# AugmentariumLab/VolumeRenderer

Hardware: AMD Instinct MI355X
Metric: Mvoxels/s kd-tree compress+decode (higher is better)
Workload: dtype u8; 1 GPU; 2048x2048x1920 uint8 volume per GPU as 960 bricks of 256x256x128, rm_volume, tolerance 1, maxEpochs 2, VolumeKdtree build + levelCut

## Files before the change

volumerenderer_amd/csrc/brickset.h:

```cpp
#pragma once
#include "kd_common.h"
#include "../../include/vrhip.h"
#include <algorithm>
#include <string>
#include <vector>

namespace vr {

struct Stream2 {
    uint8_t *temp = nullptr;
    uint8_t *codes = nullptr;
    uint8_t *recon[3] = {nullptr, nullptr, nullptr};
    Ctrl *ctrl = nullptr;
    uint8_t *tree = nullptr;
    uint8_t *treeCompact = nullptr;
};

#define EST_R0_BUDGET 8
struct Switches {
    bool decodeWalk = false;
    bool decodeFineV1 = false;
    bool decodeQuad = false;
    bool noSkipBlocks = false;
    bool noUniformBlocks = false;
    bool estExactBounds = false;
    int estBudget = EST_R0_BUDGET;
    bool pyramidBoxes = false;
    bool indexPerBlock = false;
    bool noUniformDecode = false;
};

#define VR_LOD_SLOTS 4
struct LodSlot {
    int32_t *dev = nullptr;
    int32_t *host = nullptr;
    uint8_t *idxValCut = nullptr;
    uint32_t *decTables = nullptr;
    uint8_t *rankVals = nullptr;
    int64_t *obDev = nullptr;
    int64_t *obHost = nullptr;
    vr_pool_entry *tabHost = nullptr;
    int64_t tabCap = 0;
    hipEvent_t done = nullptr;
    bool pending = false;
};

struct BrickSet {
    int32_t B = 0;
    Switches sw;
    Geom g{};
    TilePlan tile{};
    RegionPlan region{};
    Pyr12Plan pyr12{};
    int32_t D = 0, maxDepth = 0;
    int32_t tolerance = 6, maxEpochs = 5, variant = 0;
    int32_t K = 0;
    int32_t Ds = 0;
    int64_t heapStride = 0;
    int64_t leafStride = 0;
// ... 111 lines not shown
```

volumerenderer_amd/csrc/capi.hip:

```cpp
#include "../../include/vrhip.h"
#include "brickset.h"
#include "raymarch.h"
#include <math.h>
#include <stdio.h>
#include <stdlib.h>
#include <string.h>
#include <algorithm>
#include <array>
#include <atomic>
#include <map>
#include <mutex>
#include <new>

using namespace vr;

struct vr_brickset { BrickSet s; };

#define HIPCHK(x) do { hipError_t e_ = (x); if (e_ != hipSuccess) return e_ == hipErrorOutOfMemory ? VR_ERR_OOM : VR_ERR_NO_DEVICE; } while (0)

static bool device_ok()
{
    int n = 0;
    hipError_t e = hipGetDeviceCount(&n);
    if ((e != hipSuccess || n <= 0) && getenv("VRHIP_DEBUG"))
// ... 183 lines not shown
}

static bool pow2(int64_t v) { return v > 0 && (v & (v - 1)) == 0; }

static bool misaligned16(const void *p) { return ((uintptr_t)p & 15) != 0; }

vr_status vr_brickset_create(vr_brickset **out, int32_t num_bricks, const int64_t dims[3], int32_t tolerance,
                             int32_t max_epochs, int32_t variant)
{
    if (!out || !dims || num_bricks <= 0) return VR_ERR_INVALID;
    if (tolerance < 0 || max_epochs < 0 || variant < 0 || variant > 2) return VR_ERR_INVALID;
    for (int k = 0; k < 3; ++k) if (dims[k] <= 0) return VR_ERR_INVALID;
    if (max_epochs > VR_MAX_EPOCHS) return VR_ERR_UNSUPPORTED;
    bool general = !pow2(dims[0]) || !pow2(dims[1]) || !pow2(dims[2]) || dims[0] > 1024 || dims[1] > 1024 || dims[2] > 1024;
    if (dims[0] > (1ll << 20) || dims[1] > (1ll << 20) || dims[2] > (1ll << 20) || dims[0] * dims[1] * dims[2] >= (1ll << 32))
        return VR_ERR_UNSUPPORTED;
    if (num_bricks > VR_MAX_BRICKS) return VR_ERR_UNSUPPORTED;
    if (!device_ok()) return VR_ERR_NO_DEVICE;
    vr_brickset *h = new (std::nothrow) vr_brickset();
    if (!h) return VR_ERR_OOM;
    BrickSet &b = h->s;
    b.B = num_bricks;
    {
        Switches &w = b.sw;
        w.decodeWalk = getenv("VRHIP_DECODE_WALK") != nullptr;
        w.decodeFineV1 = getenv("VRHIP_DECODE_FINE_V1") != nullptr;
        w.decodeQuad = getenv("VRHIP_DECODE_QUAD") != nullptr;
        w.noSkipBlocks = getenv("VRHIP_NO_SKIP_BLOCKS") != nullptr;
        w.noUniformBlocks = getenv("VRHIP_NO_UNIFORM_BLOCKS") != nullptr;
        w.noUniformDecode = getenv("VRHIP_NO_UNIFORM_DECODE") != nullptr;
        w.pyramidBoxes = getenv("VRHIP_PYRAMID_BOXES") != nullptr;
        w.indexPerBlock = getenv("VRHIP_INDEX_PER_BLOCK") != nullptr;
        w.estExactBounds = getenv("VRHIP_EST_EXACT_BOUNDS") != nullptr;
        if (const char *eb = getenv("VRHIP_EST_BUDGET")) { const int v = atoi(eb); if (v >= 0) w.estBudget = v; }
    }
    make_geom(b.g, dims);
    b.D = b.g.D;
    if (b.D > 31) { delete h; return VR_ERR_UNSUPPORTED; }
    b.idx64 = b.D > 28 || (getenv("VRHIP_FORCE_IDX64") && b.D >= 12);
    if (b.idx64) general = true;
    if (b.idx64 && num_bricks != 1 && b.D > 28) { delete h; return VR_ERR_UNSUPPORTED; }
    b.generalGeom = general;
    b.maxDepth = b.D + VR_CHAIN_LEVELS;
    b.tolerance = tolerance; b.maxEpochs = max_epochs; b.variant = variant;
    b.K = b.D < 6 ? b.D : 6;
    b.Ds = b.D - b.K;
    b.heapStride = (int64_t)1 << (b.D + 1);
    b.leafStride = (int64_t)1 << b.D;
    b.codeStride = ((b.heapStride + 15) / 16) * 4;
    b.reconStride = b.leafStride;
    const int64_t numMax = b.heapStride - 1 + VR_CHAIN_LEVELS * b.leafStride;
    b.treeCap = ((numMax + 15) / 16 + 2) * 4 + 256;
    if (b.D >= 12) {
        const int64_t gappedBytes = ((int64_t)1 << (b.D - 12)) * 2320 * 4 + 256;
        if (gappedBytes > b.treeCap) b.treeCap = gappedBytes;
    }
    b.nIdx = (int64_t)1 << b.Ds;
    make_plans(b.g, b.K, b.generalGeom, b.idx64, b.treeCap, b.tile, b.region, b.pyr12);
    vr_status rc = alloc_stream2(b, b.mid);
    if (rc == VR_OK) {
        hipError_t e = hipMalloc(&b.idxOff, (size_t)b.B * b.nIdx * sizeof(uint32_t));
        if (e == hipSuccess) e = hipMalloc(&b.idxVal, (size_t)b.B * b.nIdx);
        if (e == hipSuccess) e = hipMalloc(&b.idxValCut, (size_t)b.B * b.nIdx);
        if (e == hipSuccess && general) {
            const int grc = build_general_geometry(&b);
            if (grc != 0) e = grc == -3 ? hipErrorOutOfMemory : hipErrorUnknown;
        }
        const auto upload = [](uint32_t *dst, const std::vector<uint32_t> &v) {
            return hipMemcpy(dst, v.data(), v.size() * sizeof(uint32_t), hipMemcpyHostToDevice);
        };
        if (e == hipSuccess) e = hipMalloc(&b.lut, ((size_t)1 << b.K) * sizeof(uint32_t));
        if (e == hipSuccess && !general) e = upload(b.lut, make_lut(b.g, b.K));
        if (e == hipSuccess && !general) e = hipMalloc(&b.spread, (size_t)(b.g.X + b.g.Y + b.g.Z) * sizeof(uint32_t));
        if (e == hipSuccess && !general) e = upload(b.spread, make_spread(b.g));
        for (int i = 0; i < 8 && e == hipSuccess; ++i) e = hipEventCreate(&b.ev[i]);
        if (e != hipSuccess) rc = e == hipErrorOutOfMemory ? VR_ERR_OOM : VR_ERR_NO_DEVICE;
    }
    if (rc != VR_OK) { vr_brickset_destroy(h); return rc; }
    b.hostCtrl.resize(b.B);
    b.openTreeBytes.assign(b.B, -1);
    *out = h;
    return VR_OK;
}

vr_status vr_brickset_set_switch(vr_brickset *h, const char *name, int32_t value)
{
    if (!h || !name) return VR_ERR_INVALID;
    Switches &w = h->s.sw;
    const bool on = value != 0;
    if (!strcmp(name, "decode_walk")) w.decodeWalk = on;
    else if (!strcmp(name, "decode_fine_v1")) w.decodeFineV1 = on;
    else if (!strcmp(name, "decode_quad")) w.decodeQuad = on;
    else if (!strcmp(name, "no_skip_blocks")) w.noSkipBlocks = on;
    else if (!strcmp(name, "no_uniform_blocks")) w.noUniformBlocks = on;
    else if (!strcmp(name, "no_uniform_decode")) w.noUniformDecode = on;
    else if (!strcmp(name, "pyramid_boxes")) w.pyramidBoxes = on;
    else if (!strcmp(name, "index_per_block")) w.indexPerBlock = on;
    else if (!strcmp(name, "est_exact_bounds")) w.estExactBounds = on;
    else return VR_ERR_INVALID;
    return VR_OK;
}

vr_status vr_brickset_set_compaction(vr_brickset *h, int32_t on_build)
{
    if (!h) return VR_ERR_INVALID;
    h->s.compactOnBuild = on_build != 0;
    return VR_OK;
}

vr_status vr_debug_set(const char *name, int32_t value)
{
    if (!name) return VR_ERR_INVALID;
    if (!strcmp(name, "skip_grid_v1")) { vr::g_skipGridV1.store(value ? 1 : 0); return VR_OK; }
    if (!strcmp(name, "reslice_tile_w")) {
        if (value != 8 && value != 16 && value != 64) return VR_ERR_INVALID;
        vr::g_resliceTileLog2.store(value == 8 ? 3 : (value == 16 ? 4 : 6));
        return VR_OK;
    }
    if (!strcmp(name, "hist_plain")) { vr::g_histPlain.store(value ? 1 : 0); return VR_OK; }
    return VR_ERR_INVALID;
}

vr_status vr_brickset_set_error_tolerance(vr_brickset *h, int32_t tol)
{
    if (!h || tol < 0) return VR_ERR_INVALID;
    h->s.tolerance = tol;
    return VR_OK;
}
vr_status vr_brickset_set_max_epochs(vr_brickset *h, int32_t e)
{
    if (!h || e < 0) return VR_ERR_INVALID;
// ... 1316 lines not shown
```

volumerenderer_amd/csrc/host_plan.cpp:

```cpp
#include "host_plan.h"
#include "../../include/vrhip.h"
#include <string.h>
#include <algorithm>
#include <atomic>
#include <thread>

namespace vr {

static int next_split(int64_t ext[3], int d)
{
    int sd = d % 3, i = 0;
    while (ext[0] * ext[1] * ext[2] > 1 && ext[sd] == 1) sd = (d + ++i) % 3;
    ext[sd] /= 2;
    return sd;
}

void make_geom(Geom &g, const int64_t dims[3])
{
    memset(&g, 0, sizeof(g));
    g.X = (int32_t)dims[0]; g.Y = (int32_t)dims[1]; g.Z = (int32_t)dims[2];
    g.voxels = dims[0] * dims[1] * dims[2];
    int64_t ext[3] = {dims[0], dims[1], dims[2]};
    for (int k = 0; k < 3; ++k) { int n = 0; while (((int64_t)1 << (n + 1)) <= dims[k]) ++n; g.nb[k] = n; }
    g.D = g.nb[0] + g.nb[1] + g.nb[2];
// ... 335 lines not shown
        if (k.numActive <= 0) return;
        const int64_t tb = (k.numActive + 3) / 4;
        std::vector<uint8_t> &r = recs[(size_t)b];
        r.assign((size_t)archive_record_bytes(g.D, g.maxDepth, tb), 0);
        uint8_t *p = r.data();
        memcpy(p, k.dmap, (size_t)g.maxDepth + 1); p += pad16(g.maxDepth + 1);
        memcpy(p, k.topVal.data(), (size_t)2 << Dc); p += pad16((int64_t)2 << Dc);
        memcpy(p, k.blockOff.data(), (size_t)4 << Dc); p += pad16((int64_t)4 << Dc);
        memcpy(p, k.tree, (size_t)tb);
        dir[(size_t)b] = ArchiveEntry{0, tb, k.numActive, fnv1a64(r.data(), (int64_t)r.size())};
    });
    int64_t at = dirEnd;
    for (int b = 0; b < g.numBricks; ++b)
        if (!recs[(size_t)b].empty()) { dir[(size_t)b].offset = at; at += (int64_t)recs[(size_t)b].size(); }
    ArchiveHeader h;
    memset(&h, 0, sizeof(h));
    memcpy(h.magic, ARCHIVE_MAGIC, 8);
    h.version = 1; h.variant = (uint32_t)g.variant; h.numBricks = g.numBricks; h.D = g.D; h.maxDepth = g.maxDepth; h.fileBytes = at;
    for (int k = 0; k < 3; ++k) h.dims[k] = g.dims[k];
    bool ok = fwrite(&h, sizeof(h), 1, f) == 1 && fwrite(dir.data(), VR_ARCHIVE_ENTRY_BYTES, dir.size(), f) == dir.size();
    for (int b = 0; ok && b < g.numBricks; ++b)
        if (!recs[(size_t)b].empty()) ok = fwrite(recs[(size_t)b].data(), 1, recs[(size_t)b].size(), f) == recs[(size_t)b].size();
    return ok;
}

bool read_header(FILE *f, Header &h)
{
    if (fread(&h, VR_HEADER_BYTES, 1, f) != 1) return false;
    return h.maxDepth >= VR_CHAIN_LEVELS && h.maxDepth < VR_MAX_DEPTH && h.numActive > 0;
}

bool write_header(FILE *f, const Header &h) { return fwrite(&h, VR_HEADER_BYTES, 1, f) == 1; }

}

extern "C" vr_status vr_lod_select_error(const vr_brick_error *table, int32_t num_bricks, int32_t cut_lo, int32_t cut_hi,
                                         int64_t voxels_per_brick, const int32_t *cuts_in, int32_t max_abs_bound,
                                         double mean_sq_bound, int32_t *cuts_out)
{
    if (!table || !cuts_out || num_bricks < 1 || cut_lo < 0 || cut_lo > cut_hi || voxels_per_brick < 1) return VR_ERR_INVALID;
    if (max_abs_bound < 0 || mean_sq_bound != mean_sq_bound) return VR_ERR_INVALID;
    for (int32_t b = 0; cuts_in && b < num_bricks; ++b) if (cuts_in[b] < -1) return VR_ERR_INVALID;
    for (int32_t b = 0; b < num_bricks; ++b) {
        const int32_t h = cuts_in ? cuts_in[b] : cut_hi;
        int32_t pick = h;
        for (int32_t c = cut_lo; h >= 0 && c <= std::min(h, cut_hi); ++c) {
            const vr_brick_error &e = table[(int64_t)(c - cut_lo) * num_bricks + b];
            if (e.max_abs > (uint32_t)max_abs_bound) continue;
            if (mean_sq_bound >= 0.0 && !((double)e.sum_sq <= mean_sq_bound * (double)voxels_per_brick)) continue;
            pick = c;
            break;
        }
        cuts_out[b] = pick;
    }
    return VR_OK;
}

extern "C" vr_status vr_stream_block_table(const int64_t dims[3], const uint8_t *tree_host, int64_t tree_bytes, int64_t num_active,
                                           const uint8_t *dmap, int32_t map_len, uint32_t *block_off_out, uint8_t *top_val_out)
{
    if (!dims || !tree_host || !dmap || !block_off_out || !top_val_out || num_active <= 0) return VR_ERR_INVALID;
    for (int k = 0; k < 3; ++k) if (dims[k] <= 0 || dims[k] > (1ll << 20)) return VR_ERR_INVALID;
    if (dims[0] * dims[1] * dims[2] >= (1ll << 32)) return VR_ERR_UNSUPPORTED;
    vr::Geom g;
    vr::make_geom(g, dims);
    if (g.D > 31 || num_active >= (1ll << 32)) return VR_ERR_UNSUPPORTED;
// ... 32 lines not shown
```

volumerenderer_amd/csrc/host_plan.h:

```cpp
#pragma once
#include <stdint.h>
#include <stdio.h>
#include <array>
#include <functional>
#include <vector>

#if defined(__HIP__) || defined(__HIPCC__)
#define VR_HD __host__ __device__
#else
#define VR_HD
#endif

#define VR_MAX_DEPTH 40
#define VR_CHAIN_LEVELS 7
#define VR_IDX_DEAD 0xFFFFFFFFu

namespace vr {

struct Geom {
    int32_t D;
    int32_t nb[3];
    int32_t X, Y, Z;
    uint8_t axis[32];
    uint8_t bit[32];
// ... 15 lines not shown
    if (code == 1) { v += dist; return v > 255 ? 255 : v; }
    if (code == 2) { v -= dist; return v < 0 ? 0 : v; }
    return v;
}

VR_HD inline int cget(const uint8_t *C, int64_t i) { return (C[i >> 2] >> ((int)(i & 3) * 2)) & 3; }

void make_geom(Geom &g, const int64_t dims[3]);
std::vector<std::array<int, 3>> split_counts(const int64_t dims[3], int depths);
std::vector<uint32_t> make_lut(const Geom &g, int K);
std::vector<uint32_t> make_spread(const Geom &g);

constexpr int VR_RG_REGX = 128;

struct TilePlan {
    bool ok;
    int jx, jy, jz, tilesX, tilesY, tilesZ, ltx, lty;
    uint8_t kqBit[8];
};
struct RegionPlan {
    bool ok;
    int X, Y, lrx, lry, jx, nreg;
    int64_t voxels;
    uint32_t lanePos, parkP[4], parkS, gAddr[4], gByte, gOut[8], xRead[2], blkX, blkY, blkZ;
};
struct Pyr12Plan {
    bool use12;
    int ax, ay, az, swz, nbx, nby, lnbx, lnby;
    uint16_t sx[16];
    bool lines;
};
void make_plans(const Geom &g, int K, bool generalGeom, bool idx64, int64_t treeCap, TilePlan &tile, RegionPlan &region,
                Pyr12Plan &pyr12);

template <class Node, class Pruned, class Chain>
int walk_stream(int D, const uint8_t *tree, int64_t numActive, const uint8_t *dmap, int cut, Node node, Pruned pruned,
                Chain chain)
{
    int v[VR_MAX_DEPTH];
    int64_t pos = 0;
    int j = 0;
    uint32_t path = 0;
    while (true) {
        if (pos >= numActive) return -1;
        const int tok = cget(tree, pos);
        const int val = j == 0 ? dmap[0] : (j <= cut ? apply_code(v[j - 1], tok, dmap[j]) : v[j - 1]);
        v[j] = val;
        node(j, path, pos++, tok, val);
        bool terminal = tok == 3;
        if (terminal) pruned(j, path, val);
        else if (j == D) {
            for (int c = 1; c <= VR_CHAIN_LEVELS; ++c) {
                if (pos >= numActive) return -2;
                chain(path);
                if (cget(tree, pos++) == 3) break;
            }
            terminal = true;
        }
        if (terminal) {
            while (j > 0 && (path & 1u)) { path >>= 1; --j; }
            if (j == 0) break;
            path |= 1u;
        } else { ++j; path <<= 1; }
    }
    return pos == numActive ? 0 : -3;
}
// ... 116 lines not shown
```

volumerenderer_amd/csrc/kd_common.h:

```cpp
#pragma once
#include <hip/hip_runtime.h>
#include "host_plan.h"

namespace vr {

struct Ctrl {
    double currentDistance, currentError, currentDF, currentStepSize;
    double previousDistance, previousError, previousDF, previousStepSize;
    unsigned long long errMinus, errPlus;
    unsigned long long statL1;
    unsigned long long numActive;
    int32_t epoch;
    int32_t active;
    int32_t fillThisEpoch;
    int32_t cur, prev, pendingEqual;
    int32_t par, ra, rb;
    int32_t numReverts;
    int32_t maxErrBefore, maxErrAfter;
    int32_t estTbase;
    unsigned long long estS;
    uint32_t estC;
    int32_t estFallbacks;
    int32_t estSeg;
    int32_t estDone;
    int32_t emitOverflow;
    int32_t constBrick;
    int32_t constVal;
    int32_t roleDist[2], codesDist, finalReconDist, finalCodesDist;
    int32_t altValid, altDist, altSel;
    int32_t zeroRun;
    uint8_t distanceMap[VR_MAX_DEPTH + 8];
};

struct Enc { int code, recon, err; };
__host__ __device__ inline Enc encode_node(int t, int p, int d)
{
    int none = p > t ? p - t : t - p;
    int add = p + d > 255 ? 255 : p + d;
    int ae = add > t ? add - t : t - add;
    int sub = p - d < 0 ? 0 : p - d;
    int se = sub > t ? sub - t : t - sub;
    int m = none < ae ? none : ae;
    m = se < m ? se : m;
    Enc e;
    e.err = m;
    if (m == none) { e.code = 0; e.recon = p; }
    else if (m == ae) { e.code = 1; e.recon = add; }
    else { e.code = 2; e.recon = sub; }
    return e;
}

#ifdef __HIPCC__
// ... 105 lines not shown
```

volumerenderer_amd/csrc/kd_encode.hip:

```cpp
#include "brickset.h"
#include <math.h>
#include <stdio.h>
#include <stdlib.h>
#include <string.h>

namespace vr {

#define FILL_NODES_PER_BLOCK 1024
#define EMIT_RANKS_PER_BLOCK 256

template <bool FROM_VOXELS>
__global__ void __launch_bounds__(256)
k_pyramid(Geom g, int dLeaf, int L, const uint8_t *__restrict__ vox, const uint8_t *__restrict__ inMin,
          const uint8_t *__restrict__ inMax, int64_t inStride, uint8_t *__restrict__ temp, int64_t heapStride,
          uint8_t *__restrict__ tempRange, uint8_t *__restrict__ outMin, uint8_t *__restrict__ outMax,
          int64_t outStride, const uint32_t *__restrict__ srcIdx)
{
    __shared__ uint8_t smn[2][1024], smx[2][1024];
    const int brick = blockIdx.y;
    const uint32_t n = 1u << L;
    const uint32_t base = blockIdx.x << L;
    uint8_t *T = temp + (int64_t)brick * heapStride;
    uint8_t *TR = tempRange ? tempRange + (int64_t)brick * heapStride : nullptr;
    for (uint32_t i = threadIdx.x; i < n; i += blockDim.x) {
// ... 357 lines not shown
    int Dm2;
};
__device__ __forceinline__ bool skip_block(const SkipBlocks &sk, int brick, int d, uint32_t node)
{
    return sk.flag && d > sk.Dm2 && (sk.flag[(int64_t)brick * sk.nBlk + (node >> (10 + d - sk.Dm2))] & 2u) != 0u;
}

#ifndef VR_FLAGS_BATCHED
#define VR_FLAGS_BATCHED 1
#endif

__device__ inline int phys_buf(const Ctrl &c, int role) { return role == 0 ? c.ra : c.rb; }

__global__ void k_ctrl_init(Ctrl *ctrls, const uint8_t *rootMin, const uint8_t *rootMax, int64_t mmStride)
{
    Ctrl &c = ctrls[blockIdx.x];
    if (threadIdx.x) return;
    c.constBrick = 0; c.constVal = 0; c.zeroRun = 0;
    if (rootMin) {
        const int mn = rootMin[(int64_t)blockIdx.x * mmStride], mx = rootMax[(int64_t)blockIdx.x * mmStride];
        c.constBrick = mn == mx ? 1 : 0;
        c.constVal = mn;
    }
    c.currentDistance = c.currentError = c.currentDF = c.currentStepSize = 0.0;
    c.previousDistance = c.previousError = c.previousDF = c.previousStepSize = 0.0;
    c.errMinus = c.errPlus = 0;
    c.statL1 = 0;
    c.numActive = 0;
    c.epoch = 0; c.active = 0; c.fillThisEpoch = 0;
    c.cur = 0; c.prev = 1; c.pendingEqual = 0;
    c.par = 0; c.ra = 1; c.rb = 2;
    c.altValid = 0; c.altSel = 0; c.altDist = 0;
    c.numReverts = 0; c.maxErrBefore = 0; c.maxErrAfter = 0;
    c.estS = 0; c.estC = 0; c.estTbase = 0; c.estFallbacks = 0; c.estSeg = 0; c.estDone = 0; c.emitOverflow = 0;
    for (int i = 0; i < VR_MAX_DEPTH + 8; ++i) c.distanceMap[i] = 0;
}

#define EST_SEG 1024
#define EST_CAND 8
#define EST_ROUNDS 5
#define EST_HEAD 4096

#define est_at(ci, seg) (((int64_t)(ci) * summStride + (int64_t)(seg)) * 4)

__device__ __forceinline__ uint32_t wave_incl_scan_u32(uint32_t v, int lane)
{
    (void)lane;
    return wave_incl_scan_add_dpp(v);
}

__device__ __forceinline__ uint32_t lane_u32(uint32_t v, int l) { return (uint32_t)__builtin_amdgcn_readlane((int)v, l); }
__device__ __forceinline__ unsigned long long lane_u64(unsigned long long v, int l)
{
    return (unsigned long long)lane_u32((uint32_t)v, l) | ((unsigned long long)lane_u32((uint32_t)(v >> 32), l) << 32);
}

#define EST_STAGE_NODES 4096
__device__ inline void est_exact_chain(const uint8_t *__restrict__ T, const uint8_t *__restrict__ P, int d, uint32_t lo,
                                       uint32_t hi, unsigned long long &S, uint32_t &C, int lane, const SkipBlocks &sk, int brick,
                                       uint8_t *stage = nullptr)
{
    const uint32_t len = hi - lo;
    const bool staged = stage && d > 0 && len >= 64u && len <= (uint32_t)EST_STAGE_NODES && (len & 63u) == 0u && (lo & 31u) == 0u;
    const uint8_t *sT = stage, *sP = stage + EST_STAGE_NODES;
    if (staged) {
        for (uint32_t i = (uint32_t)lane * 16u; i < len; i += 1024u) *(uint4 *)(stage + i) = *(const uint4 *)(T + lo + i);
        for (uint32_t i = (uint32_t)lane * 16u; i < len / 2u; i += 1024u) *(uint4 *)(stage + EST_STAGE_NODES + i) = *(const uint4 *)(P + (lo >> 1) + i);
    }
    const bool sk0 = skip_block(sk, brick, d, lo);
    int tn = 0, pn = 0;
    if (staged) { tn = sT[lane]; pn = sP[lane >> 1]; }
    else { tn = (!sk0 && lo + lane < hi) ? T[lo + lane] : 0; pn = (!sk0 && lo + lane < hi && d > 0) ? P[(lo + lane) >> 1] : 0; }
    bool skipThis = sk0;
    for (uint32_t base = lo; base < hi; base += 64) {
// ... 4 lines not shown
        {
            const uint32_t i2 = i + 64;
            skipThis = base + 64 < hi && skip_block(sk, brick, d, base + 64);
            if (staged) {
                const uint32_t j2 = i2 - lo;
                tn = j2 < len ? sT[j2] : 0;
                pn = j2 < len ? sP[j2 >> 1] : 0;
            } else {
                tn = (!skipThis && i2 < hi) ? T[i2] : 0;
                pn = (!skipThis && i2 < hi && d > 0) ? P[i2 >> 1] : 0;
            }
        }
        if (skipped) continue;
        int pd = p > t ? p - t : t - p;
        bool forced = (t > p && 2 * t - p > 255) || (t < p && 2 * t < p);
        bool cand = valid && pd > 0;
        bool dec = cand && (forced || S < (unsigned long long)pd * (2ull * C + 1ull));
        unsigned long long mask = __ballot(dec);
        for (int it = 0; it < 65; ++it) {
            uint32_t cpre = __popcll(mask & ((1ull << lane) - 1ull));
            uint32_t v = dec ? (uint32_t)pd : 0u;
            uint32_t spre = wave_incl_scan_u32(v, lane) - v;
            bool nd = cand && (forced || (S + spre) < (unsigned long long)pd * (2ull * (C + cpre) + 1ull));
            unsigned long long nmask = __ballot(nd);
            dec = nd;
            if (nmask == mask) break;
            mask = nmask;
        }
        S += (uint32_t)__builtin_amdgcn_readlane((int)wave_incl_scan_add_dpp(dec ? (uint32_t)pd : 0u), 63);
        C += __popcll(mask);
    }
}

__device__ inline int est_window_base(long long T, int nc)
{
    long long b = T - (nc <= 4 ? 1 : 2);
    if (b < 0) b = 0;
    if (b > 256 - nc) b = 256 - nc;
    return (int)b;
}

__device__ inline void est_finish(Ctrl &c, unsigned long long S, uint32_t C, int maxEpochs)
{
    c.currentDistance = C > 0 ? round((double)S / (double)C) : 0.0;
    c.previousDistance = 0.0;
    c.previousStepSize = 255.0;
    c.previousError = 65025.0;
    c.epoch = 0;
    c.active = maxEpochs > 0 ? 1 : 0;
    c.fillThisEpoch = c.active;
    c.errMinus = c.errPlus = 0;
    c.cur = 0; c.prev = 1; c.pendingEqual = 0;
}

__global__ void __launch_bounds__(64)
k_est_head(int d, int maxEpochs, Ctrl *ctrls, const uint8_t *__restrict__ temp, int64_t heapStride, ReconBufs rb,
           int64_t leafStride, SkipBlocks sk)
{
    const int brick = blockIdx.x, lane = threadIdx.x;
    Ctrl &c = ctrls[brick];
    if (c.constBrick) return;
    const uint8_t *T = temp + (int64_t)brick * heapStride + ((int64_t)1 << d);
    const uint8_t *P = rb.b[c.par] + (int64_t)brick * leafStride;
    const uint32_t n = 1u << d;
    unsigned long long S = 0;
    uint32_t C = 0;
    __shared__ __attribute__((aligned(16))) uint8_t stage[EST_STAGE_NODES + EST_STAGE_NODES / 2];
    est_exact_chain(T, P, d, 0, n < EST_HEAD ? n : EST_HEAD, S, C, lane, sk, brick, stage);
    if (lane == 0) {
        if (n <= EST_HEAD) est_finish(c, S, C, maxEpochs);
        else {
            c.estS = S; c.estC = C;
            c.estSeg = EST_HEAD / EST_SEG;
            c.estDone = 0;
            c.estTbase = est_window_base((long long)(S / (2ull * C + 1ull)), 4);
        }
    }
}

__device__ __forceinline__ uint32_t seg_incl_scan_add_dpp(uint32_t v)
{
    v = row_incl_scan_add_dpp(v);
    return v + dpp_u32<0x142, 0xa>(0, v);
}
__device__ __forceinline__ int seg_max_i32_dpp(int v)
{
    v = row_max_i32_dpp(v);
    return max(v, (int)dpp_u32<0x142, 0xa>(0x80000000u, (uint32_t)v));
}
__device__ __forceinline__ int seg_min_i32_dpp(int v)
{
    v = row_min_i32_dpp(v);
    return min(v, (int)dpp_u32<0x142, 0xa>(0x7FFFFFFFu, (uint32_t)v));
}

template <bool QUADS>
__global__ void __launch_bounds__(256)
k_est_summ(int d, int nc, Ctrl *ctrls, const uint8_t *__restrict__ temp, int64_t heapStride, ReconBufs rb,
           int64_t leafStride, uint32_t *__restrict__ summ, int64_t summStride, SkipBlocks sk)
{
    constexpr int L = 32, SPW = 64 / L, NP = EST_SEG / 2 / L, TW = NP / 2, PW = NP / 4;
    const int brick = blockIdx.y, lane = threadIdx.x & 63, row = lane / L, rl = lane % L;
    const Ctrl &c = ctrls[brick];
    const uint32_t n = 1u << d;
    const int cConst = c.constBrick, cDone = c.estDone, cSeg = c.estSeg, cPar = c.par, cTbase = c.estTbase;
    if (cConst || cDone) return;
    const uint8_t *Tl = temp + (int64_t)brick * heapStride + ((int64_t)1 << d) + rl * (4 * TW);
    const uint8_t *Pl = (cPar == 0 ? rb.b[0] : (cPar == 1 ? rb.b[1] : rb.b[2])) + (int64_t)brick * leafStride + rl * (4 * PW);
    const uint32_t nseg = n / EST_SEG, step = gridDim.x * (4u * SPW);
    const uint32_t g0 = (uint32_t)cSeg + (blockIdx.x * 4u + (threadIdx.x >> 6)) * SPW;
    uint4 tN[TW / 4], pN[PW / 4];
    auto fetch = [&](uint32_t g) {
        const uint32_t s = g + (uint32_t)row;
        const bool live = s < nseg && !skip_block(sk, brick, d, s * EST_SEG);
#pragma unroll
        for (int j = 0; j < TW / 4; ++j) tN[j] = make_uint4(0, 0, 0, 0);
#pragma unroll
        for (int j = 0; j < PW / 4; ++j) pN[j] = make_uint4(0, 0, 0, 0);
        if (live) {
#pragma unroll
            for (int j = 0; j < TW / 4; ++j) tN[j] = ld16(Tl + (size_t)s * EST_SEG + 16 * j);
#pragma unroll
            for (int j = 0; j < PW / 4; ++j) pN[j] = ld16(Pl + (size_t)s * (EST_SEG / 2) + 16 * j);
        }
    };
    fetch(g0);
    const int Tbase = cTbase;
    uint32_t *out = summ + (int64_t)brick * summStride * (4 * EST_CAND);
    for (uint32_t g = g0; g < nseg; g += step) {
    uint32_t tw[TW], pw[PW];
#pragma unroll
    for (int j = 0; j < TW / 4; ++j) { tw[4 * j] = tN[j].x; tw[4 * j + 1] = tN[j].y; tw[4 * j + 2] = tN[j].z; tw[4 * j + 3] = tN[j].w; }
#pragma unroll
    for (int j = 0; j < PW / 4; ++j) { pw[4 * j] = pN[j].x; pw[4 * j + 1] = pN[j].y; pw[4 * j + 2] = pN[j].z; pw[4 * j + 3] = pN[j].w; }
    const uint32_t seg = g + (uint32_t)row;
    const bool segLive = seg < nseg;
    uint32_t mixed = 0;
    {
        const uint32_t t0 = __builtin_amdgcn_perm(0, tw[0], 0u), p0 = __builtin_amdgcn_perm(0, pw[0], 0u);
#pragma unroll
        for (int j = 0; j < TW; ++j) mixed |= tw[j] ^ t0;
#pragma unroll
        for (int j = 0; j < PW; ++j) mixed |= pw[j] ^ p0;
    }
    const bool uniform = __ballot(mixed != 0u) == 0ull;
    constexpr int NU = QUADS ? 1 : NP, NQ = QUADS ? TW : 1;
    vr_s16x2 pd[NU], h[NU];
    uint32_t anyPd = 0;
    uint32_t pd4[NQ], hi[NQ], anyF = 0;
    vr_s16x2 pm = (vr_s16x2)(0);
    const auto unpack4 = [&](const int q) {
        const uint32_t psel = (uint32_t)((2 * q) & 3);
        const vr_s16x2 P2 = pk_s(__builtin_amdgcn_perm(0, pw[q >> 1], 0x0c000c00u | psel | ((psel + 1u) << 16)));
        const vr_s16x2 Te = pk_s(__builtin_amdgcn_perm(0, tw[q], 0x0c020c00u)), To = pk_s(__builtin_amdgcn_perm(0, tw[q], 0x0c030c01u));
        const vr_s16x2 de = Te - P2, dO = To - P2;
        const vr_s16x2 pe = __builtin_elementwise_max(de, (vr_s16x2)(0) - de), po = __builtin_elementwise_max(dO, (vr_s16x2)(0) - dO);
        const uint32_t fb = __builtin_amdgcn_perm(pk_u(To + dO), pk_u(Te + de), 0x07030501u);
        pd4[q] = __builtin_amdgcn_perm(pk_u(po), pk_u(pe), 0x06020400u);
        hi[q] = ((fb << 7) | pd4[q]) & 0x80808080u;
        anyF |= fb;
// ... 76 lines not shown
                bmin = __builtin_elementwise_min(bmin, pk_mad(cc, two2, low));
            }
        }
        } else
#pragma unroll
        for (int k = 0; k < NP; ++k) {
            const vr_s16x2 dm = (__builtin_elementwise_min(Th2, h[k]) - pd[k]) >> 15;
            low = dm * (pd[k] - w2) + low;
            cc -= dm;
            if (k < NP - 1) {
                amax = __builtin_elementwise_max(amax, low);
                bmin = __builtin_elementwise_min(bmin, pk_mad(cc, two2, low));
            }
        }
        const int low1 = low.x, low2 = low.y, cc1 = cc.x, cc2 = cc.y;
        lowT = low1 + low2; ccT = cc1 + cc2;
        a = max((int)amax.x, max((int)amax.y, 0) + low1);
        b = min((int)bmin.x, min((int)bmin.y, 0) + low1 + 2 * cc1);
        }
        const uint32_t sT = (uint32_t)(2 * Th * ccT - lowT);
        const uint32_t packed = sT | ((uint32_t)ccT << 20);
        const uint32_t incl = seg_incl_scan_add_dpp(packed), excl = incl - packed;
        const int s0 = (int)(excl & 0xFFFFFu), c0 = (int)(excl >> 20);
        a += 2 * Th * c0 - s0;
        b += 2 * (Th + 1) * c0 - s0;
        a = seg_max_i32_dpp(a);
        b = seg_min_i32_dpp(b);
        if (segLive && rl == L - 1)
            *(uint4 *)(out + est_at(ci, seg)) = make_uint4(incl & 0xFFFFFu, incl >> 20, (uint32_t)a, (uint32_t)b);
    }
    }
}

__global__ void __launch_bounds__(64)
k_est_walk(int d, int maxEpochs, int nc, int ncNext, int lastRound, int budget, Ctrl *ctrls, const uint8_t *__restrict__ temp, int64_t heapStride, ReconBufs rb,
           int64_t leafStride, const uint32_t *__restrict__ summ, int64_t summStride, SkipBlocks sk)
{
    const int brick = blockIdx.x, lane = threadIdx.x;
    Ctrl &c = ctrls[brick];
    const uint8_t *T = temp + (int64_t)brick * heapStride + ((int64_t)1 << d);
    const uint8_t *P = rb.b[c.par] + (int64_t)brick * leafStride;
    const uint32_t n = 1u << d, nseg = n / EST_SEG;
    const uint32_t *sm = summ + (int64_t)brick * summStride * (4 * EST_CAND);
    if (c.constBrick || c.estDone) return;
    __shared__ __attribute__((aligned(16))) uint8_t stage[EST_STAGE_NODES + EST_STAGE_NODES / 2];
    unsigned long long S = c.estS;
    uint32_t C = c.estC;
    const int Tbase = c.estTbase;
    long long Tc = (long long)(S / (2ull * C + 1ull));
    uint32_t seg = (uint32_t)c.estSeg;
    int fallbacks = 0;
    uint32_t preSeg = 0xFFFFFFFFu;
    long long preCi = -1;
    uint4 pre[4];
#pragma unroll
    for (int j = 0; j < 4; ++j) pre[j] = make_uint4(0, 0, 0x80000000u, 0x7FFFFFFFu);
    const auto fetch = [&](long long ci_, uint32_t seg_, uint4 (&r)[4]) {
        const uint32_t k0 = seg_ + 4u * (uint32_t)lane;
#pragma unroll
        for (int j = 0; j < 4; ++j) {
            r[j] = make_uint4(0, 0, 0x80000000u, 0x7FFFFFFFu);
            if (k0 + (uint32_t)j < nseg) r[j] = *(const uint4 *)(sm + est_at((int)ci_, k0 + (uint32_t)j));
        }
    };
    while (seg < nseg) {
        const long long ci = Tc - Tbase;
        if (ci < 0 || ci >= nc || (budget >= 0 && !lastRound && fallbacks > budget)) {
            if (!lastRound) {
                if (lane == 0) {
                    c.estS = S; c.estC = C; c.estSeg = (int)seg;
                    c.estTbase = est_window_base(Tc, ncNext);
                    c.estFallbacks += fallbacks;
                }
                return;
            }
            est_exact_chain(T, P, d, seg * EST_SEG, n, S, C, lane, sk, brick);
            fallbacks += (int)(nseg - seg);
            break;
        }
        uint4 r[4];
        if (preSeg == seg && preCi == ci) {
#pragma unroll
            for (int j = 0; j < 4; ++j) r[j] = pre[j];
        } else fetch(ci, seg, r);
        preSeg = seg + 256u; preCi = ci;
        fetch(ci, preSeg, pre);
        const uint32_t k0 = seg + 4u * (uint32_t)lane;
        const uint32_t ssL = r[0].x + r[1].x + r[2].x + r[3].x, scL = r[0].y + r[1].y + r[2].y + r[3].y;
        const uint32_t si = wave_incl_scan_u32(ssL, lane), sci = wave_incl_scan_u32(scL, lane);
        uint32_t eS = si - ssL, eC = sci - scL;
        int failJ = 4;
        uint32_t fS = 0, fC = 0;
#pragma unroll
        for (int j = 0; j < 4; ++j) {
            const long long S0 = (long long)S + (long long)eS;
            const long long q = 2ll * ((long long)C + (long long)eC) + 1ll;
            const bool ok = k0 + (uint32_t)j >= nseg || (S0 - Tc * q >= (long long)(int)r[j].z && S0 - (Tc + 1) * q < (long long)(int)r[j].w);
            if (!ok && failJ == 4) { failJ = j; fS = eS; fC = eC; }
            eS += r[j].x; eC += r[j].y;
        }
        const unsigned long long bad = __ballot(failJ < 4);
        if (bad == 0ull) {
            S += lane_u32(si, 63);
            C += lane_u32(sci, 63);
            seg += 256u;
            continue;
        }
        const int f = __ffsll((long long)bad) - 1;
        S += lane_u32(fS, f);
        C += lane_u32(fC, f);
        seg += 4u * (uint32_t)f + lane_u32((uint32_t)failJ, f);
        est_exact_chain(T, P, d, seg * EST_SEG, (seg + 1) * EST_SEG, S, C, lane, sk, brick, stage);
        Tc = (long long)(S / (2ull * C + 1ull));
        seg += 1;
        ++fallbacks;
    }
    if (lane == 0) { est_finish(c, S, C, maxEpochs); c.estFallbacks += fallbacks; c.estDone = 1; }
}

__device__ inline unsigned long long block_sum_u64(unsigned long long v, unsigned long long *sh)
{
    for (int o = 32; o > 0; o >>= 1) v += __shfl_xor(v, o);
    const int w = threadIdx.x >> 6;
    if ((threadIdx.x & 63) == 0) sh[w] = v;
    __syncthreads();
    unsigned long long r = 0;
    if (threadIdx.x == 0) for (int i = 0; i < (int)(blockDim.x >> 6); ++i) r += sh[i];
    __syncthreads();
    return r;
}

__global__ void __launch_bounds__(256)
k_fill(int d, Ctrl *ctrls, const uint8_t *__restrict__ temp, uint8_t *__restrict__ codes, int64_t heapStride,
       int64_t codeStride, ReconBufs rb, int64_t leafStride, unsigned long long *__restrict__ blockErr, int64_t nErrBlk)
{
    __shared__ unsigned long long sh[4];
    const int brick = blockIdx.y;
    Ctrl &c = ctrls[brick];
    if (c.constBrick || !c.fillThisEpoch) return;
    const uint32_t n = 1u << d;
    const uint8_t *T = temp + (int64_t)brick * heapStride + ((int64_t)1 << d);
    uint8_t *Cb = codes + (int64_t)brick * codeStride;
    const uint8_t *P = rb.b[c.par] + (int64_t)brick * leafStride;
    uint8_t *R = rb.b[phys_buf(c, c.cur)] + (int64_t)brick * leafStride;
    const int dist = (int)(uint8_t)c.currentDistance;
    const int distM = (int)(uint8_t)fmax(0.0, c.currentDistance - 1.0);
    const int distP = (int)(uint8_t)fmin(255.0, c.currentDistance + 1.0);
    unsigned long long e0 = 0, em = 0, ep = 0;
    const uint32_t i0 = (blockIdx.x * 256u + threadIdx.x) * 4u;
// ... 2030 lines not shown
    c.numReverts = 0; c.maxErrBefore = 0; c.maxErrAfter = 0; c.statL1 = 0; c.emitOverflow = 0;
}

static inline unsigned cdiv(int64_t a, int64_t b) { return (unsigned)((a + b - 1) / b); }

static void compress_stream(BrickSet *bs, Stream2 &s0, hipStream_t st, const uint8_t *rootMin, const uint8_t *rootMax,
                            int64_t mmStride, SkipBlocks sk, unsigned long long *blockErr, void *estSumm0,
                            int b0 = 0, int nb = -1)
{
    const int D = bs->D, B = nb < 0 ? bs->B : nb;
    struct { Ctrl *ctrl; uint8_t *temp, *codes; uint8_t *recon[3]; } s;
    s.ctrl = s0.ctrl + b0; s.temp = s0.temp + (int64_t)b0 * bs->heapStride; s.codes = s0.codes + (int64_t)b0 * bs->codeStride;
    for (int i = 0; i < 3; ++i) s.recon[i] = s0.recon[i] + (int64_t)b0 * bs->reconStride;
    blockErr += (int64_t)b0 * bs->nErrBlk;
    const int64_t errPlane = (int64_t)bs->B * bs->nErrBlk;
    void *estSumm = (uint32_t *)estSumm0 + (int64_t)b0 * bs->estSummStride * (4 * EST_CAND);
    if (sk.flag) sk.flag += (int64_t)b0 * sk.nBlk;
    if (rootMin) { rootMin += (int64_t)b0 * mmStride; rootMax += (int64_t)b0 * mmStride; }
    ReconBufs rb{{s.recon[0], s.recon[1], s.recon[2]}};
    const int guarded = bs->variant != 0;
    hipLaunchKernelGGL(k_ctrl_init, dim3(B), dim3(64), 0, st, s.ctrl, rootMin, rootMax, mmStride);
    if (bs->maxEpochs <= 0) {
        for (int i = 0; i < 3; ++i) hipMemsetAsync(s.recon[i], 0, (size_t)B * bs->reconStride, st);
        hipMemsetAsync(s.codes, 0, (size_t)B * bs->codeStride, st);
    }
    for (int d = 0; d <= D; ++d) {
        const int64_t n = (int64_t)1 << d;
        if (sk.flag && d == D - 1)
            hipLaunchKernelGGL(k_fill_const_leaves, dim3(cdiv(sk.nBlk, 256), B), dim3(256), 0, st, D, s.ctrl, s.temp,
                               bs->heapStride, sk);
        hipLaunchKernelGGL(k_est_head, dim3(B), dim3(64), 0, st, d, bs->maxEpochs, s.ctrl, s.temp, bs->heapStride, rb,
                           bs->reconStride, sk);
        if (n > EST_HEAD) {
            const int64_t nseg = n / EST_SEG - EST_HEAD / EST_SEG;
            for (int r = 0; r < EST_ROUNDS; ++r) {
                const int nc = r < 2 ? 4 : EST_CAND, ncNext = r + 1 < 2 ? 4 : EST_CAND;
                const unsigned gx = r == 0 ? cdiv(nseg, 32) : (cdiv(nseg, 8) < 64 ? cdiv(nseg, 8) : 64);
                const bool quads = r == 0 && !bs->sw.estExactBounds;
                hipLaunchKernelGGL(quads ? k_est_summ<true> : k_est_summ<false>, dim3(gx, B), dim3(256), 0, st, d, nc, s.ctrl, s.temp,
                                   bs->heapStride, rb, bs->reconStride, (uint32_t *)estSumm, bs->estSummStride, sk);
                hipLaunchKernelGGL(k_est_walk, dim3(B), dim3(64), 0, st, d, bs->maxEpochs, nc, ncNext,
                                   r == EST_ROUNDS - 1 ? 1 : 0, quads ? bs->sw.estBudget : -1, s.ctrl, s.temp, bs->heapStride, rb, bs->reconStride,
                                   (const uint32_t *)estSumm, bs->estSummStride, sk);
            }
        }
        for (int e = 0; e < bs->maxEpochs; ++e) {
            if (n >= 4096)
            {
                const int iters = n / 4096 >= 512 ? FILL_ITERS : (n / 4096 >= 64 ? (FILL_ITERS < 4 ? FILL_ITERS : 4) : 1);
                hipLaunchKernelGGL((bs->leafless && d == D) ? k_fill16<false> : k_fill16<true>, dim3(cdiv(n / 4096, iters), B), dim3(256), 0, st,
                                   d, bs->maxEpochs, s.ctrl, s.temp, s.codes, bs->heapStride, bs->codeStride, rb, bs->reconStride, blockErr,
                                   bs->nErrBlk, sk, errPlane, iters);
            }
            else
                hipLaunchKernelGGL(k_fill, dim3(cdiv(n, FILL_NODES_PER_BLOCK), B), dim3(256), 0, st, d, s.ctrl, s.temp,
                                   s.codes, bs->heapStride, bs->codeStride, rb, bs->reconStride, blockErr, bs->nErrBlk);
            hipLaunchKernelGGL(k_control, dim3(B), dim3(64), 0, st, d, bs->maxEpochs, guarded, s.ctrl, s.temp,
                               bs->heapStride, rb, bs->reconStride, blockErr, bs->nErrBlk, errPlane, (bs->leafless && d == D) ? 1 : 0);
        }
        hipLaunchKernelGGL(k_level_end, dim3(B), dim3(64), 0, st, d, s.ctrl);
    }
}

__global__ void k_fix_chain_distances(int D, int maxDepth, Ctrl *ctrls, Ctrl *ctrlsR)
{
    if (threadIdx.x) return;
    const int add[VR_CHAIN_LEVELS] = {64, 32, 16, 8, 4, 2, 1};
    for (int dd = D + 1, i = 0; dd <= maxDepth; ++dd, ++i) {
        ctrls[blockIdx.x].distanceMap[dd] = (uint8_t)add[i];
        if (ctrlsR) ctrlsR[blockIdx.x].distanceMap[dd] = (uint8_t)add[i];
    }
}

static bool dbg_sync(hipStream_t st, const char *phase)
{
// ... 243 lines not shown
```

Measured before the change: 315,400 Mvoxels/s.

## Replace fixed estimate rounds with prefix-staged quad schedule and shared fallback budget

```diff
diff --git a/volumerenderer_amd/csrc/brickset.h b/volumerenderer_amd/csrc/brickset.h
--- a/volumerenderer_amd/csrc/brickset.h
+++ b/volumerenderer_amd/csrc/brickset.h
@@ -16,7 +16,7 @@
     uint8_t *treeCompact = nullptr;
 };
 
-#define EST_R0_BUDGET 8
+#define EST_QUAD_BUDGET 8
 struct Switches {
     bool decodeWalk = false;
     bool decodeFineV1 = false;
@@ -24,7 +24,8 @@
     bool noSkipBlocks = false;
     bool noUniformBlocks = false;
     bool estExactBounds = false;
-    int estBudget = EST_R0_BUDGET;
+    bool estOldSchedule = false;
+    int estBudget = EST_QUAD_BUDGET;
     bool pyramidBoxes = false;
     bool indexPerBlock = false;
     bool noUniformDecode = false;
diff --git a/volumerenderer_amd/csrc/capi.hip b/volumerenderer_amd/csrc/capi.hip
--- a/volumerenderer_amd/csrc/capi.hip
+++ b/volumerenderer_amd/csrc/capi.hip
@@ -239,6 +239,7 @@
         w.pyramidBoxes = getenv("VRHIP_PYRAMID_BOXES") != nullptr;
         w.indexPerBlock = getenv("VRHIP_INDEX_PER_BLOCK") != nullptr;
         w.estExactBounds = getenv("VRHIP_EST_EXACT_BOUNDS") != nullptr;
+        w.estOldSchedule = getenv("VRHIP_EST_OLD_SCHEDULE") != nullptr;
         if (const char *eb = getenv("VRHIP_EST_BUDGET")) { const int v = atoi(eb); if (v >= 0) w.estBudget = v; }
     }
     make_geom(b.g, dims);
@@ -304,6 +305,7 @@
     else if (!strcmp(name, "pyramid_boxes")) w.pyramidBoxes = on;
     else if (!strcmp(name, "index_per_block")) w.indexPerBlock = on;
     else if (!strcmp(name, "est_exact_bounds")) w.estExactBounds = on;
+    else if (!strcmp(name, "est_old_schedule")) w.estOldSchedule = on;
     else return VR_ERR_INVALID;
     return VR_OK;
 }
diff --git a/volumerenderer_amd/csrc/host_plan.cpp b/volumerenderer_amd/csrc/host_plan.cpp
--- a/volumerenderer_amd/csrc/host_plan.cpp
+++ b/volumerenderer_amd/csrc/host_plan.cpp
@@ -391,6 +391,29 @@
 
 bool write_header(FILE *f, const Header &h) { return fwrite(&h, VR_HEADER_BYTES, 1, f) == 1; }
 
+EstPlan est_round_plan(uint32_t nseg, bool oldSchedule)
+{
+    constexpr uint32_t first = VR_EST_HEAD / VR_EST_SEG, EST_MIN_PREFIX = 8;
+    EstPlan p{};
+    const auto add = [&](uint32_t end, int nc, bool quads, int sweeps = 4) { p.r[p.rounds++] = EstRound{end, nc, quads, sweeps}; };
+    if (nseg <= first) return p;
+    if (oldSchedule) {
+        add(nseg, 4, true);
+        add(nseg, 4, false);
+    } else {
+        const uint32_t len = nseg - first;
+        uint32_t at = first;
+        for (const int shift : {4, 2}) {
+            const uint32_t pre = len >> shift;
+            if (pre >= EST_MIN_PREFIX && first + pre > at) { at = first + pre; add(at, shift == 4 ? 4 : 2, true); }
+        }
+        add(nseg, 1, true);
+        add(nseg, 4, true, 16);
+    }
+    for (int i = 0; i < 3; ++i) add(nseg, VR_EST_CAND, false);
+    return p;
+}
+
 }
 
 extern "C" vr_status vr_lod_select_error(const vr_brick_error *table, int32_t num_bricks, int32_t cut_lo, int32_t cut_hi,
diff --git a/volumerenderer_amd/csrc/host_plan.h b/volumerenderer_amd/csrc/host_plan.h
--- a/volumerenderer_amd/csrc/host_plan.h
+++ b/volumerenderer_amd/csrc/host_plan.h
@@ -71,6 +71,18 @@
 };
 void make_plans(const Geom &g, int K, bool generalGeom, bool idx64, int64_t treeCap, TilePlan &tile, RegionPlan &region,
                 Pyr12Plan &pyr12);
+
+constexpr int VR_EST_SEG = 1024, VR_EST_HEAD = 4096, VR_EST_CAND = 8, VR_EST_MAX_ROUNDS = 8;
+struct EstRound { uint32_t segEnd; int32_t nc; bool quads; int32_t sweeps; };
+struct EstPlan { int32_t rounds; EstRound r[VR_EST_MAX_ROUNDS]; };
+EstPlan est_round_plan(uint32_t nseg, bool oldSchedule);
+VR_HD inline int est_window_base(long long T, int up, int nc)
+{
+    long long b = T - (nc >= 8 ? 2 : (nc >= 3 ? 1 : (nc == 2 && !up ? 1 : 0)));
+    if (b < 0) b = 0;
+    if (b > 256 - nc) b = 256 - nc;
+    return (int)b;
+}
 
 template <class Node, class Pruned, class Chain>
 int walk_stream(int D, const uint8_t *tree, int64_t numActive, const uint8_t *dmap, int cut, Node node, Pruned pruned,
diff --git a/volumerenderer_amd/csrc/kd_common.h b/volumerenderer_amd/csrc/kd_common.h
--- a/volumerenderer_amd/csrc/kd_common.h
+++ b/volumerenderer_amd/csrc/kd_common.h
@@ -17,7 +17,9 @@
     int32_t par, ra, rb;
     int32_t numReverts;
     int32_t maxErrBefore, maxErrAfter;
-    int32_t estTbase;
+    int32_t estT;
+    int32_t estUp;
+    int32_t estQuadFb;
     unsigned long long estS;
     uint32_t estC;
     int32_t estFallbacks;
diff --git a/volumerenderer_amd/csrc/kd_encode.hip b/volumerenderer_amd/csrc/kd_encode.hip
--- a/volumerenderer_amd/csrc/kd_encode.hip
+++ b/volumerenderer_amd/csrc/kd_encode.hip
@@ -413,14 +413,13 @@
     c.par = 0; c.ra = 1; c.rb = 2;
     c.altValid = 0; c.altSel = 0; c.altDist = 0;
     c.numReverts = 0; c.maxErrBefore = 0; c.maxErrAfter = 0;
-    c.estS = 0; c.estC = 0; c.estTbase = 0; c.estFallbacks = 0; c.estSeg = 0; c.estDone = 0; c.emitOverflow = 0;
+    c.estS = 0; c.estC = 0; c.estT = 0; c.estUp = 0; c.estQuadFb = 0; c.estFallbacks = 0; c.estSeg = 0; c.estDone = 0; c.emitOverflow = 0;
     for (int i = 0; i < VR_MAX_DEPTH + 8; ++i) c.distanceMap[i] = 0;
 }
 
-#define EST_SEG 1024
-#define EST_CAND 8
-#define EST_ROUNDS 5
-#define EST_HEAD 4096
+#define EST_SEG VR_EST_SEG
+#define EST_CAND VR_EST_CAND
+#define EST_HEAD VR_EST_HEAD
 
 #define est_at(ci, seg) (((int64_t)(ci) * summStride + (int64_t)(seg)) * 4)
 
@@ -491,12 +490,12 @@
     }
 }
 
-__device__ inline int est_window_base(long long T, int nc)
-{
-    long long b = T - (nc <= 4 ? 1 : 2);
-    if (b < 0) b = 0;
-    if (b > 256 - nc) b = 256 - nc;
-    return (int)b;
+__device__ inline void est_park(Ctrl &c, unsigned long long S, uint32_t C, uint32_t seg)
+{
+    const unsigned long long q = 2ull * C + 1ull, T = S / q;
+    c.estS = S; c.estC = C; c.estSeg = (int)seg;
+    c.estT = (int)T;
+    c.estUp = 2ull * (S - T * q) >= q ? 1 : 0;
 }
 
 __device__ inline void est_finish(Ctrl &c, unsigned long long S, uint32_t C, int maxEpochs)
@@ -529,10 +528,9 @@
     if (lane == 0) {
         if (n <= EST_HEAD) est_finish(c, S, C, maxEpochs);
         else {
-            c.estS = S; c.estC = C;
-            c.estSeg = EST_HEAD / EST_SEG;
+            est_park(c, S, C, EST_HEAD / EST_SEG);
             c.estDone = 0;
-            c.estTbase = est_window_base((long long)(S / (2ull * C + 1ull)), 4);
+            c.estQuadFb = 0;
         }
     }
 }
@@ -555,18 +553,18 @@
 
 template <bool QUADS>
 __global__ void __launch_bounds__(256)
-k_est_summ(int d, int nc, Ctrl *ctrls, const uint8_t *__restrict__ temp, int64_t heapStride, ReconBufs rb,
+k_est_summ(int d, int nc, uint32_t segEnd, int budget, Ctrl *ctrls, const uint8_t *__restrict__ temp, int64_t heapStride, ReconBufs rb,
            int64_t leafStride, uint32_t *__restrict__ summ, int64_t summStride, SkipBlocks sk)
 {
     constexpr int L = 32, SPW = 64 / L, NP = EST_SEG / 2 / L, TW = NP / 2, PW = NP / 4;
     const int brick = blockIdx.y, lane = threadIdx.x & 63, row = lane / L, rl = lane % L;
     const Ctrl &c = ctrls[brick];
-    const uint32_t n = 1u << d;
-    const int cConst = c.constBrick, cDone = c.estDone, cSeg = c.estSeg, cPar = c.par, cTbase = c.estTbase;
-    if (cConst || cDone) return;
+    const int cConst = c.constBrick, cDone = c.estDone, cSeg = c.estSeg, cPar = c.par, cT = c.estT, cUp = c.estUp, cFb = c.estQuadFb;
+    if (cConst || cDone || (budget >= 0 && cFb > budget)) return;
+    const uint32_t nseg = segEnd;
     const uint8_t *Tl = temp + (int64_t)brick * heapStride + ((int64_t)1 << d) + rl * (4 * TW);
     const uint8_t *Pl = (cPar == 0 ? rb.b[0] : (cPar == 1 ? rb.b[1] : rb.b[2])) + (int64_t)brick * leafStride + rl * (4 * PW);
-    const uint32_t nseg = n / EST_SEG, step = gridDim.x * (4u * SPW);
+    const uint32_t step = gridDim.x * (4u * SPW);
     const uint32_t g0 = (uint32_t)cSeg + (blockIdx.x * 4u + (threadIdx.x >> 6)) * SPW;
     uint4 tN[TW / 4], pN[PW / 4];
     auto fetch = [&](uint32_t g) {
@@ -584,7 +582,7 @@
         }
     };
     fetch(g0);
-    const int Tbase = cTbase;
+    const int Tbase = est_window_base(cT, cUp, nc);
     uint32_t *out = summ + (int64_t)brick * summStride * (4 * EST_CAND);
     for (uint32_t g = g0; g < nseg; g += step) {
     uint32_t tw[TW], pw[PW];
@@ -727,8 +725,30 @@
     }
 }
 
+#ifdef VR_EST_CENSUS
+#define EST_CENSUS_CAP (1u << 22)
+__device__ uint32_t g_estCensusN;
+__device__ uint4 g_estCensus[EST_CENSUS_CAP];
+enum { EC_WALKED = 1, EC_WINDOW = 2, EC_BUDGET = 3, EC_LIMIT = 4, EC_DONE = 5, EC_LAST_RESORT = 6, EC_START = 7 };
+#define EST_UP(S_, C_, T_) (2ull * ((S_) - (unsigned long long)(T_) * (2ull * (C_) + 1ull)) >= 2ull * (C_) + 1ull ? 256u : 0u)
+#define EST_LOG(kind, seg_, T_) do { if (lane == 0) { const uint32_t i_ = atomicAdd(&g_estCensusN, 1u); \
+    if (i_ < EST_CENSUS_CAP) g_estCensus[i_] = make_uint4((uint32_t)brick | ((uint32_t)d << 16) | ((uint32_t)round << 24), (seg_), (uint32_t)(T_), (kind)); } } while (0)
+extern "C" int64_t vr_debug_est_census(uint32_t *out, int64_t capRecords)
+{
+    uint32_t n = 0, zero = 0;
+    if (hipDeviceSynchronize() != hipSuccess || hipMemcpyFromSymbol(&n, HIP_SYMBOL(g_estCensusN), 4) != hipSuccess) return -1;
+    const int64_t m = n < EST_CENSUS_CAP ? n : EST_CENSUS_CAP;
+    if (m > capRecords) return -2;
+    if (m && hipMemcpyFromSymbol(out, HIP_SYMBOL(g_estCensus), (size_t)m * 16) != hipSuccess) return -1;
+    if (hipMemcpyToSymbol(HIP_SYMBOL(g_estCensusN), &zero, 4) != hipSuccess) return -1;
+    return n;
+}
+#else
+#define EST_LOG(kind, seg_, T_) do { } while (0)
+#endif
+
 __global__ void __launch_bounds__(64)
-k_est_walk(int d, int maxEpochs, int nc, int ncNext, int lastRound, int budget, Ctrl *ctrls, const uint8_t *__restrict__ temp, int64_t heapStride, ReconBufs rb,
+k_est_walk(int d, int maxEpochs, int nc, uint32_t segEnd, int round, int lastRound, int budget, Ctrl *ctrls, const uint8_t *__restrict__ temp, int64_t heapStride, ReconBufs rb,
            int64_t leafStride, const uint32_t *__restrict__ summ, int64_t summStride, SkipBlocks sk)
 {
     const int brick = blockIdx.x, lane = threadIdx.x;
@@ -738,13 +758,16 @@
     const uint32_t n = 1u << d, nseg = n / EST_SEG;
     const uint32_t *sm = summ + (int64_t)brick * summStride * (4 * EST_CAND);
     if (c.constBrick || c.estDone) return;
+    const int fb0 = c.estQuadFb;
+    if (budget >= 0 && fb0 > budget) return;
     __shared__ __attribute__((aligned(16))) uint8_t stage[EST_STAGE_NODES + EST_STAGE_NODES / 2];
     unsigned long long S = c.estS;
     uint32_t C = c.estC;
-    const int Tbase = c.estTbase;
+    const int Tbase = est_window_base(c.estT, c.estUp, nc);
     long long Tc = (long long)(S / (2ull * C + 1ull));
     uint32_t seg = (uint32_t)c.estSeg;
     int fallbacks = 0;
+    EST_LOG(EC_START | EST_UP(S, C, Tc), seg, Tc);
     uint32_t preSeg = 0xFFFFFFFFu;
     long long preCi = -1;
     uint4 pre[4];
@@ -755,22 +778,29 @@
 #pragma unroll
         for (int j = 0; j < 4; ++j) {
             r[j] = make_uint4(0, 0, 0x80000000u, 0x7FFFFFFFu);
-            if (k0 + (uint32_t)j < nseg) r[j] = *(const uint4 *)(sm + est_at((int)ci_, k0 + (uint32_t)j));
+            if (k0 + (uint32_t)j < segEnd) r[j] = *(const uint4 *)(sm + est_at((int)ci_, k0 + (uint32_t)j));
         }
     };
-    while (seg < nseg) {
+    const auto park = [&]() {
+        if (lane == 0) {
+            est_park(c, S, C, seg);
+            c.estFallbacks += fallbacks;
+            if (budget >= 0) c.estQuadFb = fb0 + fallbacks;
+        }
+    };
+    while (seg < segEnd) {
         const long long ci = Tc - Tbase;
-        if (ci < 0 || ci >= nc || (budget >= 0 && !lastRound && fallbacks > budget)) {
+        const bool spent = budget >= 0 && !lastRound && fb0 + fallbacks > budget;
+        if (ci < 0 || ci >= nc || spent) {
             if (!lastRound) {
-                if (lane == 0) {
-                    c.estS = S; c.estC = C; c.estSeg = (int)seg;
-                    c.estTbase = est_window_base(Tc, ncNext);
-                    c.estFallbacks += fallbacks;
-                }
+                EST_LOG(spent ? EC_BUDGET : EC_WINDOW, seg, Tc);
+                park();
                 return;
             }
+            EST_LOG(EC_LAST_RESORT, seg, Tc);
             est_exact_chain(T, P, d, seg * EST_SEG, n, S, C, lane, sk, brick);
             fallbacks += (int)(nseg - seg);
+            seg = nseg;
             break;
         }
         uint4 r[4];
@@ -790,7 +820,7 @@
         for (int j = 0; j < 4; ++j) {
             const long long S0 = (long long)S + (long long)eS;
             const long long q = 2ll * ((long long)C + (long long)eC) + 1ll;
-            const bool ok = k0 + (uint32_t)j >= nseg || (S0 - Tc * q >= (long long)(int)r[j].z && S0 - (Tc + 1) * q < (long long)(int)r[j].w);
+            const bool ok = k0 + (uint32_t)j >= segEnd || (S0 - Tc * q >= (long long)(int)r[j].z && S0 - (Tc + 1) * q < (long long)(int)r[j].w);
             if (!ok && failJ == 4) { failJ = j; fS = eS; fC = eC; }
             eS += r[j].x; eC += r[j].y;
         }
@@ -798,7 +828,7 @@
         if (bad == 0ull) {
             S += lane_u32(si, 63);
             C += lane_u32(sci, 63);
-            seg += 256u;
+            seg = seg + 256u < segEnd ? seg + 256u : segEnd;
             continue;
         }
         const int f = __ffsll((long long)bad) - 1;
@@ -809,7 +839,14 @@
         Tc = (long long)(S / (2ull * C + 1ull));
         seg += 1;
         ++fallbacks;
-    }
+        EST_LOG(EC_WALKED | EST_UP(S, C, Tc), seg - 1u, Tc);
+    }
+    if (seg < nseg) {
+        EST_LOG(EC_LIMIT, seg, Tc);
+        park();
+        return;
+    }
+    EST_LOG(EC_DONE, seg, Tc);
     if (lane == 0) { est_finish(c, S, C, maxEpochs); c.estFallbacks += fallbacks; c.estDone = 1; }
 }
 
@@ -2906,15 +2943,17 @@
         hipLaunchKernelGGL(k_est_head, dim3(B), dim3(64), 0, st, d, bs->maxEpochs, s.ctrl, s.temp, bs->heapStride, rb,
                            bs->reconStride, sk);
         if (n > EST_HEAD) {
-            const int64_t nseg = n / EST_SEG - EST_HEAD / EST_SEG;
-            for (int r = 0; r < EST_ROUNDS; ++r) {
-                const int nc = r < 2 ? 4 : EST_CAND, ncNext = r + 1 < 2 ? 4 : EST_CAND;
-                const unsigned gx = r == 0 ? cdiv(nseg, 32) : (cdiv(nseg, 8) < 64 ? cdiv(nseg, 8) : 64);
-                const bool quads = r == 0 && !bs->sw.estExactBounds;
-                hipLaunchKernelGGL(quads ? k_est_summ<true> : k_est_summ<false>, dim3(gx, B), dim3(256), 0, st, d, nc, s.ctrl, s.temp,
-                                   bs->heapStride, rb, bs->reconStride, (uint32_t *)estSumm, bs->estSummStride, sk);
-                hipLaunchKernelGGL(k_est_walk, dim3(B), dim3(64), 0, st, d, bs->maxEpochs, nc, ncNext,
-                                   r == EST_ROUNDS - 1 ? 1 : 0, quads ? bs->sw.estBudget : -1, s.ctrl, s.temp, bs->heapStride, rb, bs->reconStride,
+            const vr::EstPlan plan = vr::est_round_plan((uint32_t)(n / EST_SEG), bs->sw.estOldSchedule);
+            for (int r = 0; r < plan.rounds; ++r) {
+                const vr::EstRound &R = plan.r[r];
+                const int64_t len = (int64_t)R.segEnd - EST_HEAD / EST_SEG;
+                const unsigned gx = R.quads ? cdiv(len, 8 * R.sweeps) : (cdiv(len, 8) < 64 ? cdiv(len, 8) : 64);
+                const bool quads = R.quads && !bs->sw.estExactBounds;
+                const int budget = quads ? bs->sw.estBudget : -1;
+                hipLaunchKernelGGL(quads ? k_est_summ<true> : k_est_summ<false>, dim3(gx, B), dim3(256), 0, st, d, R.nc, R.segEnd, budget,
+                                   s.ctrl, s.temp, bs->heapStride, rb, bs->reconStride, (uint32_t *)estSumm, bs->estSummStride, sk);
+                hipLaunchKernelGGL(k_est_walk, dim3(B), dim3(64), 0, st, d, bs->maxEpochs, R.nc, R.segEnd, r,
+                                   r == plan.rounds - 1 ? 1 : 0, budget, s.ctrl, s.temp, bs->heapStride, rb, bs->reconStride,
                                    (const uint32_t *)estSumm, bs->estSummStride, sk);
             }
         }
```

After: 328,000 Mvoxels/s (median of 6 runs). +4.0%, better.
